# visinf/style-seqcvae

Measured on AMD Instinct MI355X. Metric: captions/sec (train step), higher is better.
Workload: dtype f32; 1 GPU; C2 train step: fwd+bwd+allreduce+clip+SGD, B=64/GPU, R=36, F=2048, L=20 (T=21), Z=128, V=10000, E=1000, H=1200, A=768, SENTIMENT_VAE=1; global_batch=64, parallelism=dp1

## Files before the change

### include/ssc.h

```cpp
#ifndef SSC_H
#define SSC_H

#include <stddef.h>
#include <stdint.h>

#ifdef __cplusplus
extern "C" {
#endif

#define SSC_OK 0
#define SSC_EINVAL (-1)
#define SSC_EALIGN (-2)
#define SSC_EHIP (-3)
#define SSC_EWORKSPACE (-4)

#define SSC_MAX_SEG 6

int ssc_version(void);
int ssc_last_hip_error(void);
const char* ssc_arch(void);

typedef struct {
  const float* A; const float* B;
  int lda, ldb, K;
// ... 14 lines not shown
  const int* m_count; const int* a_rows; const int* c_rows;
  const int* k_count; const int* ka_rows; const int* kb_rows;
  const float* a_scale; const float* b_scale;
  float* topk_part;
} ssc_gemm_desc;

int ssc_pow2_scale(const float* x, size_t rows, int cols, size_t ld, int target_log2, float* out, int combine, float* scratch,
                   void* stream);

int ssc_split_f16(const float* x, int rows, int K, int ldx, const float* scale, void* out, int ldo, const int* row_list,
                  const int* row_count, void* stream);

int ssc_gemm(const ssc_gemm_desc* d, void* stream);

int ssc_gemm_dw_group(const ssc_gemm_desc* const* d, int n, void* stream);

int ssc_set_gemm_mode(int mode);
int ssc_gemm_auto_splits(int M, int N, int ksteps);

int ssc_feat_prep(const float* feats, int B, int R, int F, float* mask, float* avg, void* stream);

int ssc_prep_tokens(const int64_t* caps, int B, int L, int pad, int boundary, int64_t* tokens_tm, float* w_tm,
                    float* nvalid, void* stream);

int ssc_embed_gather(const float* table, int ldt, const int64_t* ids, int n, int E, float* out, int ldo, void* stream);
int ssc_embed_scatter_add(float* dtable, int ldt, const int64_t* ids, int n, int E, const float* d, int ldd, int pad,
                          void* stream);

typedef struct {
  int B, H;
// ... 548 lines not shown
```

### include/ssc_debug.h

```cpp
#ifndef SSC_DEBUG_H
#define SSC_DEBUG_H

#ifdef __cplusplus
extern "C" {
#endif

int ssc_prof_enable(int on);
int ssc_prof_collect(float* out, int max_records);

int ssc_prof_loop_enable(int on);
int ssc_prof_loop_ms(float* fwd_loop_ms, float* bwd_loop_ms);

int ssc_debug_set(const char* key, int value);
int ssc_debug_get(const char* key, int* value);

#ifdef __cplusplus
}
#endif
#endif
```

### style-seqcvae_amd/csrc/gemm.hip

```cpp
#include <stdio.h>
#include <stdlib.h>
#include <string.h>

#include "ssc_common.h"
#include "ssc_debug.h"

typedef float f32x16 __attribute__((ext_vector_type(16)));

namespace {

constexpr int BM = 64, BN = 64, BK = 32;
constexpr int KC_LD = BK + 4;

struct KSeg {
  const float* A;
  const float* B;
  int lda, ldb, K, nsteps;
  int avec, bvec;
  const float* A16;
  const float* B16;
  int lda16, ldb16;
};

struct KArgs {
// ... 1489 lines not shown
    a.seg.s.A16 = a.seg.s.B16 = nullptr; a.seg.s.lda16 = a.seg.s.ldb16 = 0;
    a.nseg = 1; a.M = m.M; a.N = m.N;
    a.out = m.C; a.ldo = m.ldc; a.slab_stride = 0; a.bias = nullptr; a.accumulate = m.accumulate;
    a.steps_total = a.steps_per_split = a.seg.s.nsteps;
    a.mcount = a.arows = a.crows = nullptr;
    a.kcount = m.kcount; a.karows = m.karows; a.kbrows = m.kbrows;
    a.tile_gm = g.tile_gm; a.store_wt = g.store_wt; a.member = p;
    a.topk = nullptr; a.a_scale = a.b_scale = nullptr;
    const int gx = (m.N + 127) / 128, gy = (m.M + 127) / 128;
    const int local = t - m.first;
    x3w_body<false, false, true, 128, 128, PF, NPW>(a, local % gx, local / gx, 0, gx, gy, 1, thr);
    __syncthreads();
  }
}

__global__ void reduce_slabs_kernel(const float* __restrict__ slabs, int nslab, size_t slab_stride, int M, int N,
                                    float* __restrict__ C, int ldc, const float* __restrict__ bias, int accumulate,
                                    const int* __restrict__ mcount, const int* __restrict__ crows) {
  size_t i = (size_t)blockIdx.x * blockDim.x + threadIdx.x;
  if (mcount) M = min(M, *mcount);
  size_t total = (size_t)M * N;
  if (i >= total) return;
  int row = (int)(i / N), col = (int)(i % N);
  float v = 0.f;
  for (int s0 = 0; s0 < nslab; s0 += 8) {
    float t[8];
#pragma unroll
    for (int u = 0; u < 8; ++u) t[u] = slabs[(size_t)min(s0 + u, nslab - 1) * slab_stride + i];
#pragma unroll
    for (int u = 0; u < 8; ++u) v += (s0 + u < nslab) ? t[u] : 0.f;
// ... 198 lines not shown
enum { X3W_NT, X3W_NN, X3W_TN, X3W_TN_KG, X3W_NT_F16_4, X3W_NT_F16_8, X3W_SKINNY_NT, X3W_SKINNY_NN, X3W_FORMS };
const X3wForm g_x3w[X3W_FORMS] = {
    x3w_form<true, true, false, 128, 128, 2, 8>("128x128"), x3w_form<true, false, false, 128, 128, 2, 8>("128x128"),
    x3w_form<false, false, false, 128, 128, 2, 8>("128x128"), x3w_form<false, false, true, 128, 128, 1, 8>("128x128"),
    x3w_form<true, true, false, 128, 128, 2, 4, true>("128x128 f16"), x3w_form<true, true, false, 128, 128, 2, 8, true>("128x128 f16"),
    x3w_form<true, true, false, 64, 256, 2, 8>("64x256"), x3w_form<true, false, false, 64, 256, 2, 8>("64x256"),
};
inline const X3wForm& x3w_big(bool a_kc, bool b_kc, bool kg) {
  return g_x3w[(a_kc && b_kc) ? X3W_NT : a_kc ? X3W_NN : kg ? X3W_TN_KG : X3W_TN];
}
inline const X3wForm& x3w_skinny_form(bool b_kc) { return g_x3w[b_kc ? X3W_SKINNY_NT : X3W_SKINNY_NN]; }

typedef void (*tn_list_fn)(const KTnList);
const tn_list_fn g_tn_list_fn = gemm_x3w_kernel_tn_list<1, 8>;
constexpr int TN_LIST_THREADS = 256 + 64 * 8, TN_LIST_LDS = x3w_lds_bytes<128, 128>();
int g_cus[64] = {};

int x3w_prepare() {
  static bool done_dev[64] = {};
  int dev = 0;
  if (hipGetDevice(&dev) != hipSuccess || dev < 0 || dev >= 64) return SSC_EHIP;
  bool& done = done_dev[dev];
  if (done) return SSC_OK;
  for (const X3wForm& f : g_x3w)
    if (hipFuncSetAttribute((const void*)f.fn, hipFuncAttributeMaxDynamicSharedMemorySize, f.lds) != hipSuccess) return SSC_EHIP;
  if (hipFuncSetAttribute((const void*)g_tn_list_fn, hipFuncAttributeMaxDynamicSharedMemorySize, TN_LIST_LDS) != hipSuccess) return SSC_EHIP;
  if (hipDeviceGetAttribute(&g_cus[dev], hipDeviceAttributeMultiprocessorCount, dev) != hipSuccess || g_cus[dev] < 1) return SSC_EHIP;
  done = true;
  return SSC_OK;
}

inline bool x3w_span_ok(const ssc_gemm_desc* d) {
  const size_t lim = (size_t)1 << 30;
  if (d->ka_rows || d->kb_rows)
    for (int i = 0; i < d->nseg; ++i)
      if (d->seg[i].lda >= (1 << 22) || d->seg[i].ldb >= (1 << 22) || d->seg[i].K >= (1 << 24)) return false;
  for (int i = 0; i < d->nseg; ++i) {
    const size_t K = (size_t)d->seg[i].K;
    if (K == 0) continue;
    const size_t sa = d->a_kc ? (size_t)(d->M - 1) * d->seg[i].lda + K : (K - 1) * d->seg[i].lda + d->M;
    const size_t sb = d->b_kc ? (size_t)(d->N - 1) * d->seg[i].ldb + K : (K - 1) * d->seg[i].ldb + d->N;
// ... 6 lines not shown
}
inline bool vec_all(const KArgs& k) {
  for (int i = 0; i < k.nseg; ++i)
    if (!k.seg[i].avec || !k.seg[i].bvec) return false;
  return true;
}
inline bool x3w_ok(const ssc_gemm_desc* d, const KArgs& k, Num num) {
  return num != Num::F32 && vec_all(k) && (d->a_kc || !d->b_kc) && x3w_span_ok(d);
}

struct Form {
  gemm_fn fn = nullptr;
  const X3wForm* x3w = nullptr;
  dim3 grid;
};
int plan(const ssc_gemm_desc* d, const KArgs& k, int splits, Num num, Form& f) {
  const bool x3 = num != Num::F32, vec = vec_all(k);
  const bool mlist = k.mcount || k.arows || k.crows, klist = k.kcount || k.karows || k.kbrows;
  const bool compact = mlist || klist;
  if (k.topk && !(x3 && vec && d->a_kc && d->b_kc && splits == 1 && !klist && x3w_span_ok(d))) return SSC_EINVAL;
  if (compact) {
    if (!vec) return SSC_EALIGN;
    if (!x3 || (!d->a_kc && d->b_kc)) return SSC_EINVAL;
    if (klist && (k.nseg != 1 || d->a_kc || d->b_kc)) return SSC_EINVAL;
    if (mlist && !d->a_kc) return SSC_EINVAL;
  }
  if (!compact && !k.topk && x3w_skinny_layout(d) && x3w_skinny_shape(d->M, d->N, num) && x3w_ok(d, k, num)) {
    f.x3w = &x3w_skinny_form(d->b_kc);
    f.grid = dim3(ssc_cdiv(d->N, 256), ssc_cdiv(d->M, 64), splits);
    return SSC_OK;
  }
  if (x3 && vec && (d->a_kc || !d->b_kc) && (compact || k.topk || (g_x3b && big_tile(d->M, d->N)))) {
    f.grid = dim3(ssc_cdiv(d->N, 128), ssc_cdiv(d->M, 128), splits);
    const bool kg = k.karows || k.kbrows;
    const long wgs = (long)f.grid.x * f.grid.y * f.grid.z;
    const bool f16 = num == Num::X3_F16 && d->a_kc && d->b_kc && !kg && g_x3b != 3;
    const bool x3w = k.topk || g_x3b == 2 || (g_x3b == 1 && (f16 || wgs >= 768 || (d->M < 512 && big_tile(d->M, d->N))));
    if (x3w && x3w_span_ok(d) && (!kg || (k.karows && k.kbrows))) {
      f.x3w = f16 ? &g_x3w[g_f16_npw == 4 ? X3W_NT_F16_4 : X3W_NT_F16_8] : &x3w_big(d->a_kc, d->b_kc, kg);
      return SSC_OK;
    }
    f.fn = (d->a_kc && d->b_kc) ? gemm_x3b_kernel<true, true, false>
           : d->a_kc            ? gemm_x3b_kernel<true, false, false>
           : kg                 ? gemm_x3b_kernel<false, false, true>
                                : gemm_x3b_kernel<false, false, false>;
    return SSC_OK;
  }
  if (x3 && vec && d->a_kc && d->b_kc) {
    f.fn = gemm_x3_kernel;
    f.grid = dim3(ssc_cdiv(d->N, 64), ssc_cdiv(d->M, 64), splits);
    return SSC_OK;
  }
// ... 332 lines not shown
    *reinterpret_cast<u32x2*>(o + 16) = lo;
  }
}
}
extern "C" int ssc_split_f16(const float* x, int rows, int K, int ldx, const float* scale, void* out, int ldo, const int* row_list,
                             const int* row_count, void* stream) {
  const int kp = ssc_cdiv(K, BK) * BK;
  if (!x || !out || rows <= 0 || K <= 0 || ldx < K || ldo < kp || (ldo & 3) || !ssc_aligned16(out) || (row_list != nullptr) != (row_count != nullptr))
    return SSC_EINVAL;
  SSC_LAUNCH(split_f16_kernel, dim3(ssc_cdiv(kp / 4, 256), rows < 65535 ? rows : 65535), dim3(256), 0, (hipStream_t)stream, x, rows, K, ldx, scale,
             static_cast<unsigned*>(out), ldo, row_list, row_count);
  SSC_CHECK_LAUNCH();
  return SSC_OK;
}

extern "C" int ssc_gemm(const ssc_gemm_desc* d, void* stream) {
  hipStream_t st = (hipStream_t)stream;
  KArgs k;
  SSC_TRY(build_args(d, k));
  if (d->topk_part) {
    k.out = nullptr; k.ldo = d->N; k.slab_stride = 0; k.bias = d->bias; k.accumulate = 0;
    return launch(d, k, 1, st);
  }
  if (!d->C || d->ldc < d->N) return SSC_EINVAL;
  int splits = d->splits;
  if (splits <= 0) splits = ssc_gemm_auto_splits(d->M, d->N, k.steps_total);
  if (splits > k.steps_total) splits = k.steps_total;
  {
    int per = ssc_cdiv(k.steps_total, splits);
    splits = ssc_cdiv(k.steps_total, per);
  }
  if (splits > 1 && (!d->workspace || d->workspace_floats < (size_t)splits * d->M * d->N)) {
    if (d->splits > 1) return SSC_EWORKSPACE;
    splits = d->workspace ? (int)(d->workspace_floats / ((size_t)d->M * d->N)) : 1;
    if (splits < 1) splits = 1;
    int per = ssc_cdiv(k.steps_total, splits);
    splits = ssc_cdiv(k.steps_total, per);
  }
  if (splits == 1) {
    k.out = d->C;
    k.ldo = d->ldc;
    k.slab_stride = 0;
    k.bias = d->bias;
    k.accumulate = d->accumulate;
    return launch(d, k, 1, st);
  }
  k.out = d->workspace;
  k.ldo = d->N;
  k.slab_stride = (size_t)d->M * d->N;
  k.bias = nullptr;
  k.accumulate = 0;
  k.crows = nullptr;
  SSC_TRY(launch(d, k, splits, st));
  size_t total = (size_t)d->M * d->N;
  SSC_LAUNCH(reduce_slabs_kernel, dim3((unsigned)((total + 255) / 256)), dim3(256), 0, st, d->workspace, splits,
                     k.slab_stride, d->M, d->N, d->C, d->ldc, d->bias, d->accumulate, d->m_count, d->c_rows);
  SSC_CHECK_LAUNCH();
  return SSC_OK;
}

extern "C" int ssc_prof_enable(int on) {
  if (on && !g_prof) {
    g_prof = new ProfRec[PROF_MAX];
    for (int i = 0; i < PROF_MAX; ++i) {
      if (hipEventCreate(&g_prof[i].e0) != hipSuccess || hipEventCreate(&g_prof[i].e1) != hipSuccess) return SSC_EHIP;
    }
  }
  if (on && !g_prof_counts && hipHostMalloc((void**)&g_prof_counts, PROF_SLOTS * sizeof(int), hipHostMallocDefault) != hipSuccess) return SSC_EHIP;
  g_prof_on = on != 0;
  if (on) { g_prof_n = 0; g_prof_slots = 0; }
  return SSC_OK;
}
// ... 28 lines not shown
  if (mode == 0 || mode == 1) g_gemm_mode = mode;
  return prev;
}

extern int ssc_g_dec_att_table, ssc_g_dec_dedup, ssc_g_beam_reg, ssc_g_dec_ungathered, ssc_g_dec_parts, ssc_g_dec_planes;
extern int ssc_g_img_mfma;
extern int ssc_g_dw_one_flush;
extern int ssc_g_stream_nt;
namespace {
struct DebugKey { const char* name; int* var; };
const DebugKey g_debug_keys[] = {
    {"large_form", &g_x3b},
    {"x3w_skinny", &g_x3w_skinny},
    {"store_wt", &g_store_wt},
    {"tile_gm", &g_tile_gm},
    {"dw_one_flush", &ssc_g_dw_one_flush},
    {"dec_dedup", &ssc_g_dec_dedup},
    {"beam_reg", &ssc_g_beam_reg},
    {"img_mfma", &ssc_g_img_mfma},
    {"dec_ungathered", &ssc_g_dec_ungathered},
    {"dec_planes", &ssc_g_dec_planes},
    {"dec_parts", &ssc_g_dec_parts},
    {"dec_att_table", &ssc_g_dec_att_table},
    {"f16_npw", &g_f16_npw},
    {"stream_nt", &ssc_g_stream_nt},
    {"gemm_f16", &g_gemm_f16},
};
}

extern "C" int ssc_debug_set(const char* key, int value) {
// ... 20 lines not shown
```

### style-seqcvae_amd/csrc/sequence.hip

```cpp
#include <cstdlib>
#include <initializer_list>

#include "sample_draw.h"
#include "ssc_common.h"
#include "ssc_debug.h"

namespace {

inline size_t r4(size_t x) { return (x + 3) & ~(size_t)3; }

struct Layout {
  int B, R, L, T;
  int V, E, H, A, F, Z, S, tied;
  int Ep, Hp, Ap, Fp, Zp, Vp, H4, XW;
  int D, Dp, SC, NX;
  size_t wc_e, wc_d, pool, dpm;
  size_t total = 0;
  size_t act;
  size_t live;
  size_t tok, w, nvalid, sent_all, wcol_e, wcol_d, mask, avg, pv, emb, ga_static, ga_avg;
  size_t h1, c1, he, ce, hd, cd, gates_a, gates_e, gates_d, q, attn_logits, alpha, att, mu, lv, z, mulv;
  size_t slabs, slab_floats, logits, lse, proj;
  size_t nllw0, nll;
  size_t kld_raw, fb_kdim, fb_gdim, fb_gstep, fb_acc;
// ... 135 lines not shown
  ssc_gemm_desc d;
  fill_desc(d, true, b_kc, segs, M, N);
  d.C = C; d.ldc = ldc; d.bias = bias; d.accumulate = 0;
  d.splits = 0;
  d.workspace = c.slabs; d.workspace_floats = c.slab_floats;
  if (c.act_rows) {
    const int* cnt = live ? c.live_count : c.act_count;
    const int* rows = live ? c.live_rows : c.act_rows;
    d.m_count = cnt; d.a_rows = rows; d.c_rows = rows;
    const int rc = ssc_gemm(&d, c.st);
    if (rc != SSC_EALIGN && rc != SSC_EINVAL) return rc;
    d.m_count = d.a_rows = d.c_rows = nullptr;
  }
  return ssc_gemm(&d, c.st);
}
struct DwBatch {
  static constexpr int MAX = 24;
  ssc_gemm_desc d[MAX];
  int n = 0;
};
int queue_dw(const Ctx& c, DwBatch& q, const float* A, int lda, const float* Bm, int ldb, int K, int M, int N, float* C, int ldc) {
  if (q.n >= DwBatch::MAX) return SSC_EINVAL;
  ssc_gemm_desc& d = q.d[q.n++];
  fill_desc(d, false, false, {{A, lda, Bm, ldb, K}}, M, N);
  d.C = C; d.ldc = ldc;
  d.splits = 0;
  d.workspace = c.slabs; d.workspace_floats = c.slab_floats;
  if (c.live_rows) { d.k_count = c.live_count; d.ka_rows = c.live_rows; d.kb_rows = c.live_rows; }
  return SSC_OK;
}
// ... 252 lines not shown
  Ctx c{st, W + l.slabs, l.slab_floats};
  const int B = l.B, R = l.R, T = l.T, E = l.E, H = l.H, A = l.A, F = l.F, Z = l.Z, S = l.S, V = l.V, H4 = l.H4;
  const int TB = T * B;
  int64_t* tok = (int64_t*)(W + l.tok);
  const size_t sH = (size_t)B * l.Hp;
  const bool fb_on = free_bits > 0.f;

  SSC_TRY(ssc_prep_tokens(bt->caps, B, l.L, cfg->pad, cfg->boundary, tok, W + l.w, W + l.nvalid, st));
  int* act = (int*)(W + l.act);
  int* live = (int*)(W + l.live);
  SSC_LAUNCH(build_active_rows_kernel, dim3(2), dim3(1024), 0, st, W + l.w, TB, B, act, live);
  SSC_CHECK_LAUNCH();
  c.act_count = act; c.act_rows = act + 4;
  c.live_count = live; c.live_rows = live + 4;
  SSC_TRY(ssc_feat_prep(bt->feats, B, R, F, W + l.mask, W + l.avg, st));
  SSC_TRY(gemm(c, true, true, {{bt->feats, F, p->wv, p->ld_wv, F}}, B * R, A, W + l.pv, A));
  const int hoisted = ss_on ? B : TB;
  SSC_TRY(ssc_embed_gather(p->emb, p->ld_emb, tok, hoisted, E, W + l.emb, l.Ep, st));
  SSC_TRY(gemm(c, true, true, {{W + l.emb, l.Ep, p->att_w_ih, p->ld_att_w_ih, E}}, hoisted, H4, W + l.ga_static, H4));
  int64_t* fed_ids = (int64_t*)(W + l.fed_ids);
  if (ss_on && hipMemcpyAsync(fed_ids, tok, (size_t)B * sizeof(int64_t), hipMemcpyDeviceToDevice, st) != hipSuccess) return SSC_EHIP;
  SSC_TRY(gemm(c, true, true, {{W + l.avg, F, p->att_w_ih + E, p->ld_att_w_ih, F}}, B, H4, W + l.ga_avg, H4));
  {
    FillList f;
    for (size_t off : {l.h1, l.c1, l.he, l.ce, l.hd, l.cd}) f.add(W + off, sH);
    f.add(kld, (size_t)B);
    if (fb_on) {
      f.add(W + l.kld_raw, (size_t)B);
      if (free_bits_mode == 3) f.add(W + l.fb_acc, (size_t)B * l.Zp);
    }
    if (l.Zp != Z) {
      f.add(W + l.z, (size_t)TB * l.Zp); f.add(W + l.mu, (size_t)TB * l.Zp); f.add(W + l.lv, (size_t)TB * l.Zp);
    }
    if (cfg->tied) f.add(W + l.proj, (size_t)TB * l.Ep);
// ... 462 lines not shown
  }

  if (g_loop.on) { (void)hipEventRecord(g_loop.e[3], st); g_loop.bwd = true; }

  if (S == 1 && !l.D) {
    SSC_LAUNCH(repeat_kernel, dim3(ssc_cdiv(TB, 256)), dim3(256), 0, st, bt->sentiment, B, T, W + l.sent_all);
    SSC_CHECK_LAUNCH();
  }
  }

  const int zcol = F + 2 * H + S;
  const float* dga = W + l.dga; const float* dge = W + l.dge; const float* dgd = W + l.dgd;
  const float* h1_prev = W + l.h1; const float* h1_new = W + l.h1 + sH;
  const float* hd_prev = W + l.hd; const float* he_prev = W + l.he; const float* he_new = W + l.he + sH;
  const float* att = W + l.att;
  if (phases & 64u) {
  if (g->emb && !cfg->tied) {
    SSC_TRY(ssc_fill(W + l.demb, (size_t)TB * l.Ep, 0.f, st));
    SSC_TRY(gemm_rows(c, false, {{dga, H4, p->att_w_ih, p->ld_att_w_ih, H4}}, TB, E, W + l.demb, l.Ep, nullptr, true));
    if (hipMemset2DAsync(g->emb, (size_t)g->ld_emb * sizeof(float), 0, (size_t)E * sizeof(float), V, st) != hipSuccess)
      return SSC_EHIP;
    SSC_TRY(ssc_embed_scatter_add(g->emb, g->ld_emb, fed_inputs ? (const int64_t*)(W + l.fed_ids) : tok, TB, E, W + l.demb, l.Ep,
                                  cfg->pad, st));
  }
  }
  auto queue_att = [&](DwBatch& q) -> int {
    if (g->att_w_ih) {
      float* gw = g->att_w_ih; int ld = g->ld_att_w_ih;
      SSC_TRY(queue_dw(c, q, dga, H4, W + l.emb, l.Ep, TB, H4, E, gw, ld));
      SSC_TRY(queue_dw(c, q, dga, H4, h1_prev, l.Hp, TB, H4, H, gw + E + F, ld));
      SSC_TRY(queue_dw(c, q, dga, H4, hd_prev, l.Hp, TB, H4, H, gw + E + F + H, ld));
    } else if (g->att_w_hh) {
      SSC_TRY(queue_dw(c, q, dga, H4, h1_prev, l.Hp, TB, H4, H, g->att_w_hh, g->ld_att_w_hh));
    }
    if (g->wq) SSC_TRY(queue_dw(c, q, W + l.dq, l.Ap, h1_new, l.Hp, TB, A, H, g->wq, g->ld_wq));
    return SSC_OK;
  };
  auto queue_enc = [&](DwBatch& q) -> int {
// ... 29 lines not shown
      SSC_TRY(queue_dw(c, q, dgd, H4, hd_prev, l.Hp, TB, H4, H, g->dec_w_hh, g->ld_dec_w_hh));
    }
    return SSC_OK;
  };
  if (one_flush) {
    SSC_TRY(queue_att(dwq));
    SSC_TRY(queue_enc(dwq));
    SSC_TRY(queue_dec(dwq));
    SSC_TRY(flush_dw(c, dwq));
  }
  if (phases & 128u) {
  if (!one_flush) {
    SSC_TRY(queue_att(dwq));
    SSC_TRY(flush_dw(c, dwq));
  }
  if (g->att_w_ih) {
    float* gw = g->att_w_ih; int ld = g->ld_att_w_ih;
    SSC_TRY(gemm(c, false, false, {{W + l.dga_sum, H4, W + l.avg, F, B}}, H4, F, gw + E, ld));
  }
  if (g->att_w_hh) {
    if (g->att_w_ih) {
      if (hipMemcpy2DAsync(g->att_w_hh, (size_t)g->ld_att_w_hh * sizeof(float), g->att_w_ih + E + F,
                           (size_t)g->ld_att_w_ih * sizeof(float), (size_t)H * sizeof(float), H4, hipMemcpyDeviceToDevice,
                           st) != hipSuccess)
        return SSC_EHIP;
    }
  }
  if (g->att_b_ih && g->att_b_hh) {
    SSC_TRY(ssc_colsum2(dga, H4, TB, H4, nullptr, g->att_b_ih, 1, g->att_b_hh, 0, c.slabs, st));
  } else {
    if (g->att_b_ih) SSC_TRY(ssc_colsum2(dga, H4, TB, H4, nullptr, g->att_b_ih, 1, nullptr, 0, c.slabs, st));
    if (g->att_b_hh) SSC_TRY(ssc_colsum2(dga, H4, TB, H4, nullptr, g->att_b_hh, 1, nullptr, 0, c.slabs, st));
  }
  if (g->wv) SSC_TRY(gemm(c, false, false, {{W + l.dpv, A, bt->feats, F, B * R}}, A, F, g->wv, g->ld_wv));
  if (g->wa) SSC_TRY(ssc_colsum(W + l.dwa, A, B, A, nullptr, g->wa, 1, 0, st));
  }
  if (phases & 4u) {
  if (!one_flush) {
    SSC_TRY(queue_enc(dwq));
    SSC_TRY(flush_dw(c, dwq));
  }
  if (g->enc_w_ih) {
    float* gw = g->enc_w_ih; int ld = g->ld_enc_w_ih;
    if (S == 1 && !l.D) SSC_TRY(ssc_colsum2(dge, H4, TB, H4, W + l.sent_all, gw + F + 2 * H, ld, nullptr, 0, c.slabs, st));
    if (l.D && hipMemcpy2DAsync(gw + F + 2 * H, (size_t)ld * sizeof(float), W + l.wc_e, (size_t)l.Dp * sizeof(float),
                                (size_t)l.SC * sizeof(float), H4, hipMemcpyDeviceToDevice, st) != hipSuccess)
      return SSC_EHIP;
  }
  if (g->enc_b_ih && g->enc_b_hh) {
// ... 81 lines not shown
```

### style-seqcvae_amd/ssc_runtime/lib.py

```python
import ctypes as C
import os

_HERE = os.path.dirname(os.path.abspath(__file__))
DEBUG_ENV = os.environ.get("SSC_DEBUG", "") == "1"
LIB_PATH = (DEBUG_ENV and os.environ.get("SSC_LIB_PATH")) or os.path.join(os.path.dirname(_HERE), "libssc_hip.so")
SSC_MAX_SEG = 6

c_float_p = C.POINTER(C.c_float)
c_i64_p = C.POINTER(C.c_int64)
vp = C.c_void_p


class SscError(RuntimeError):
    CODES = {-1: "SSC_EINVAL", -2: "SSC_EALIGN", -3: "SSC_EHIP", -4: "SSC_EWORKSPACE"}

    def __init__(self, fn, rc, hip=0):
        super().__init__(f"{fn} failed: {self.CODES.get(rc, rc)}" + (f" (hipError {hip})" if rc == -3 else ""))
        self.rc = rc


class GemmSeg(C.Structure):
    _fields_ = [("A", vp), ("B", vp), ("lda", C.c_int), ("ldb", C.c_int), ("K", C.c_int),
                ("A16", vp), ("B16", vp), ("lda16", C.c_int), ("ldb16", C.c_int)]

# ... 174 lines not shown

class ScstDesc(C.Structure):
    _fields_ = [("P", C.c_int), ("N", C.c_int), ("steps", C.c_int), ("L", C.c_int), ("end_index", C.c_int), ("predictions", vp),
                ("scores", vp), ("base_scores", vp), ("reward_weights", C.c_double * 6), ("baseline", C.c_int),
                ("loss_scale", C.c_double), ("kld_scale", C.c_double), ("caps", vp), ("lengths", vp), ("reward", vp),
                ("advantage", vp), ("gl", vp), ("gk", vp), ("stats", vp)]


_i, _f, _sz = C.c_int, C.c_float, C.c_size_t
SYMBOLS = {
    "ssc_version": (_i, []),
    "ssc_last_hip_error": (_i, []),
    "ssc_arch": (C.c_char_p, []),
    "ssc_gemm": (_i, [C.POINTER(GemmDesc), vp]),
    "ssc_gemm_dw_group": (_i, [C.POINTER(C.POINTER(GemmDesc)), _i, vp]),
    "ssc_gemm_auto_splits": (_i, [_i, _i, _i]),
    "ssc_pow2_scale": (_i, [vp, _sz, _i, _sz, _i, vp, _i, vp, vp]),
    "ssc_split_f16": (_i, [vp, _i, _i, _i, vp, vp, _i, vp, vp, vp]),
    "ssc_decode_planes_ld": (_i, [vp]),
    "ssc_set_gemm_mode": (_i, [_i]),
    "ssc_feat_prep": (_i, [vp, _i, _i, _i, vp, vp, vp]),
    "ssc_prep_tokens": (_i, [vp, _i, _i, _i, _i, vp, vp, vp, vp]),
    "ssc_embed_gather": (_i, [vp, _i, vp, _i, _i, vp, _i, vp]),
    "ssc_embed_scatter_add": (_i, [vp, _i, vp, _i, _i, vp, _i, _i, vp]),
    "ssc_lstm_fwd": (_i, [C.POINTER(LstmFwdDesc), vp]),
    "ssc_lstm_fwd_z": (_i, [C.POINTER(LstmFwdDesc), vp, _i, vp, _i, _i, vp]),
    "ssc_lstm_fwd_p": (_i, [C.POINTER(LstmFwdDesc), vp, _i, _i, vp, vp]),
    "ssc_lstm_fwd_img": (_i, [C.POINTER(LstmFwdDesc), vp, _i, vp, _i, _i, vp]),
    "ssc_lstm_bwd_x": (_i, [C.POINTER(LstmBwdDesc), vp, _i, vp, _i, _i, vp]),
    "ssc_lstm_bwd": (_i, [C.POINTER(LstmBwdDesc), vp]),
# ... 104 lines not shown
    "ssc_eval_score": (_i, [C.POINTER(EvalRefs), C.POINTER(EvalScoreDesc), vp, _sz, vp]),
    "ssc_eval_set_workspace_bytes": (_sz, [C.POINTER(EvalRefs), C.POINTER(EvalSetDesc)]),
    "ssc_eval_set": (_i, [C.POINTER(EvalRefs), C.POINTER(EvalSetDesc), vp, _sz, vp]),
    "ssc_l2_normalize_rows": (_i, [vp, _i, _i, _i, vp, _i, vp]),
    "ssc_knn_merge": (_i, [vp, _i, _i, _i, _i, _i, vp, vp, vp, vp]),
    "ssc_eval_consensus_workspace_bytes": (_sz, [C.POINTER(EvalRefs), C.POINTER(EvalConsensusDesc)]),
    "ssc_eval_consensus": (_i, [C.POINTER(EvalRefs), C.POINTER(EvalConsensusDesc), vp, _sz, vp]),
    "ssc_scst_prepare": (_i, [C.POINTER(ScstDesc), vp]),
}

DEBUG_SYMBOLS = {
    "ssc_prof_enable": (_i, [_i]),
    "ssc_prof_collect": (_i, [vp, _i]),
    "ssc_prof_loop_enable": (_i, [_i]),
    "ssc_prof_loop_ms": (_i, [C.POINTER(C.c_float), C.POINTER(C.c_float)]),
    "ssc_debug_set": (_i, [C.c_char_p, _i]),
    "ssc_debug_get": (_i, [C.c_char_p, C.POINTER(C.c_int)]),
}

_lib = None


class _Lib:
    def __init__(self, cdll):
        self._cdll = cdll
        for name, (res, args) in list(SYMBOLS.items()) + list(DEBUG_SYMBOLS.items()):
            fn = getattr(cdll, name)
            fn.restype = res
            fn.argtypes = args
            setattr(self, "_raw_" + name, fn)
# ... 39 lines not shown
```

Before: 7996 captions/s.

## Batch independent large GEMMs into one persistent grouped list kernel

Adds a grouped GEMM list kernel that runs several independent large x3w 128x128 GEMMs in one persistent launch, with tiles ordered by steps per split. It is used for the forward visual-projection and embedding-input GEMMs and for three backward weight-gradient GEMMs (embedding grad, att_w_ih avg part, wv). The aim is to cut launch count and fill the CUs better when single GEMMs underfill the device. In exchange it forces the x3w form for listed GEMMs, carves split-K workspace per member, and moves the embedding scatter later in the backward pass.

```diff
diff --git a/include/ssc.h b/include/ssc.h
--- a/include/ssc.h
+++ b/include/ssc.h
@@ -52,6 +52,8 @@
 int ssc_gemm(const ssc_gemm_desc* d, void* stream);
 
 int ssc_gemm_dw_group(const ssc_gemm_desc* const* d, int n, void* stream);
+
+int ssc_gemm_list(const ssc_gemm_desc* const* d, int n, void* stream);
 
 int ssc_set_gemm_mode(int mode);
 int ssc_gemm_auto_splits(int M, int N, int ksteps);
diff --git a/include/ssc_debug.h b/include/ssc_debug.h
--- a/include/ssc_debug.h
+++ b/include/ssc_debug.h
@@ -1,5 +1,7 @@
 #ifndef SSC_DEBUG_H
 #define SSC_DEBUG_H
+
+#include "ssc.h"
 
 #ifdef __cplusplus
 extern "C" {
@@ -11,6 +13,8 @@
 int ssc_prof_loop_enable(int on);
 int ssc_prof_loop_ms(float* fwd_loop_ms, float* bwd_loop_ms);
 
+int ssc_debug_list_plan(const ssc_gemm_desc* const* d, int n, int* out);
+
 int ssc_debug_set(const char* key, int value);
 int ssc_debug_get(const char* key, int* value);
 
diff --git a/style-seqcvae_amd/csrc/gemm.hip b/style-seqcvae_amd/csrc/gemm.hip
--- a/style-seqcvae_amd/csrc/gemm.hip
+++ b/style-seqcvae_amd/csrc/gemm.hip
@@ -1527,6 +1527,37 @@
   }
 }
 
+enum { LIST_NT = 0, LIST_NN = 1, LIST_TN = 2, LIST_TN_KG = 3 };
+struct KList {
+  KArgs a[SSC_GROUP_MAX];
+  int n, total;
+  int first[SSC_GROUP_MAX + 1];
+  int gx[SSC_GROUP_MAX], gy[SSC_GROUP_MAX], gz[SSC_GROUP_MAX], lay[SSC_GROUP_MAX];
+};
+template <int NPW>
+__global__ __launch_bounds__(256 + 64 * NPW, 1) void gemm_x3w_kernel_list(const KList g) {
+  int p = 0;
+  for (int t = blockIdx.x; t < g.total; t += gridDim.x) {
+#pragma unroll 1
+    while (p + 1 < g.n && t >= g.first[p + 1]) ++p;
+    int thr = (int)threadIdx.x;
+    asm volatile("" : "+v"(thr));
+    __builtin_assume(thr >= 0 && thr < 256 + 64 * NPW);
+    const KArgs& a = g.a[p];
+    const int gx = g.gx[p], gy = g.gy[p], gz = g.gz[p];
+    const int local = t - g.first[p];
+    const int x = local % gx, yz = local / gx;
+    const int y = yz % gy, z = yz / gy;
+    switch (g.lay[p]) {
+      case LIST_NT: x3w_body<true, true, false, 128, 128, 2, NPW>(a, x, y, z, gx, gy, gz, thr); break;
+      case LIST_NN: x3w_body<true, false, false, 128, 128, 2, NPW>(a, x, y, z, gx, gy, gz, thr); break;
+      case LIST_TN: x3w_body<false, false, false, 128, 128, 2, NPW>(a, x, y, z, gx, gy, gz, thr); break;
+      default: x3w_body<false, false, true, 128, 128, 1, NPW>(a, x, y, z, gx, gy, gz, thr); break;
+    }
+    __syncthreads();
+  }
+}
+
 __global__ void reduce_slabs_kernel(const float* __restrict__ slabs, int nslab, size_t slab_stride, int M, int N,
                                     float* __restrict__ C, int ldc, const float* __restrict__ bias, int accumulate,
                                     const int* __restrict__ mcount, const int* __restrict__ crows) {
@@ -1755,6 +1786,8 @@
 typedef void (*tn_list_fn)(const KTnList);
 const tn_list_fn g_tn_list_fn = gemm_x3w_kernel_tn_list<1, 8>;
 constexpr int TN_LIST_THREADS = 256 + 64 * 8, TN_LIST_LDS = x3w_lds_bytes<128, 128>();
+typedef void (*list_fn)(const KList);
+const list_fn g_list_fn = gemm_x3w_kernel_list<8>;
 int g_cus[64] = {};
 
 int x3w_prepare() {
@@ -1766,6 +1799,7 @@
   for (const X3wForm& f : g_x3w)
     if (hipFuncSetAttribute((const void*)f.fn, hipFuncAttributeMaxDynamicSharedMemorySize, f.lds) != hipSuccess) return SSC_EHIP;
   if (hipFuncSetAttribute((const void*)g_tn_list_fn, hipFuncAttributeMaxDynamicSharedMemorySize, TN_LIST_LDS) != hipSuccess) return SSC_EHIP;
+  if (hipFuncSetAttribute((const void*)g_list_fn, hipFuncAttributeMaxDynamicSharedMemorySize, TN_LIST_LDS) != hipSuccess) return SSC_EHIP;
   if (hipDeviceGetAttribute(&g_cus[dev], hipDeviceAttributeMultiprocessorCount, dev) != hipSuccess || g_cus[dev] < 1) return SSC_EHIP;
   done = true;
   return SSC_OK;
@@ -1802,7 +1836,8 @@
   const X3wForm* x3w = nullptr;
   dim3 grid;
 };
-int plan(const ssc_gemm_desc* d, const KArgs& k, int splits, Num num, Form& f) {
+int plan(const ssc_gemm_desc* d, const KArgs& k, int splits, Num num, Form& f, int large_form = -1) {
+  const int x3b = large_form >= 0 ? large_form : g_x3b;
   const bool x3 = num != Num::F32, vec = vec_all(k);
   const bool mlist = k.mcount || k.arows || k.crows, klist = k.kcount || k.karows || k.kbrows;
   const bool compact = mlist || klist;
@@ -1818,12 +1853,12 @@
     f.grid = dim3(ssc_cdiv(d->N, 256), ssc_cdiv(d->M, 64), splits);
     return SSC_OK;
   }
-  if (x3 && vec && (d->a_kc || !d->b_kc) && (compact || k.topk || (g_x3b && big_tile(d->M, d->N)))) {
+  if (x3 && vec && (d->a_kc || !d->b_kc) && (compact || k.topk || (x3b && big_tile(d->M, d->N)))) {
     f.grid = dim3(ssc_cdiv(d->N, 128), ssc_cdiv(d->M, 128), splits);
     const bool kg = k.karows || k.kbrows;
     const long wgs = (long)f.grid.x * f.grid.y * f.grid.z;
-    const bool f16 = num == Num::X3_F16 && d->a_kc && d->b_kc && !kg && g_x3b != 3;
-    const bool x3w = k.topk || g_x3b == 2 || (g_x3b == 1 && (f16 || wgs >= 768 || (d->M < 512 && big_tile(d->M, d->N))));
+    const bool f16 = num == Num::X3_F16 && d->a_kc && d->b_kc && !kg && x3b != 3;
+    const bool x3w = k.topk || x3b == 2 || (x3b == 1 && (f16 || wgs >= 768 || (d->M < 512 && big_tile(d->M, d->N))));
     if (x3w && x3w_span_ok(d) && (!kg || (k.karows && k.kbrows))) {
       f.x3w = f16 ? &g_x3w[g_f16_npw == 4 ? X3W_NT_F16_4 : X3W_NT_F16_8] : &x3w_big(d->a_kc, d->b_kc, kg);
       return SSC_OK;
@@ -2186,6 +2221,110 @@
   return SSC_OK;
 }
 
+int ssc_g_large_list = ssc_env_int("SSC_LARGE_LIST", 1);
+namespace {
+int resolve_output(const ssc_gemm_desc* d, KArgs& k, int& splits) {
+  if (!d->C || d->ldc < d->N) return SSC_EINVAL;
+  splits = d->splits;
+  if (splits <= 0) splits = ssc_gemm_auto_splits(d->M, d->N, k.steps_total);
+  if (splits > k.steps_total) splits = k.steps_total;
+  {
+    int per = ssc_cdiv(k.steps_total, splits);
+    splits = ssc_cdiv(k.steps_total, per);
+  }
+  if (splits > 1 && (!d->workspace || d->workspace_floats < (size_t)splits * d->M * d->N)) {
+    if (d->splits > 1) return SSC_EWORKSPACE;
+    splits = d->workspace ? (int)(d->workspace_floats / ((size_t)d->M * d->N)) : 1;
+    if (splits < 1) splits = 1;
+    int per = ssc_cdiv(k.steps_total, splits);
+    splits = ssc_cdiv(k.steps_total, per);
+  }
+  if (splits == 1) {
+    k.out = d->C;
+    k.ldo = d->ldc;
+    k.slab_stride = 0;
+    k.bias = d->bias;
+    k.accumulate = d->accumulate;
+    return SSC_OK;
+  }
+  k.out = d->workspace;
+  k.ldo = d->N;
+  k.slab_stride = (size_t)d->M * d->N;
+  k.bias = nullptr;
+  k.accumulate = 0;
+  k.crows = nullptr;
+  return SSC_OK;
+}
+int reduce_output(const ssc_gemm_desc* d, const KArgs& k, int splits, hipStream_t st) {
+  size_t total = (size_t)d->M * d->N;
+  SSC_LAUNCH(reduce_slabs_kernel, dim3((unsigned)((total + 255) / 256)), dim3(256), 0, st, d->workspace, splits,
+                     k.slab_stride, d->M, d->N, d->C, d->ldc, d->bias, d->accumulate, d->m_count, d->c_rows);
+  SSC_CHECK_LAUNCH();
+  return SSC_OK;
+}
+
+inline bool ranges_overlap(const float* a, size_t na, const float* b, size_t nb) { return a < b + nb && b < a + na; }
+int list_layout(const ssc_gemm_desc* d, const KArgs& k, int splits, Num num) {
+  if (num != Num::X3 || g_x3b == 0 || g_x3b == 3 || k.topk || d->M < BIG_MIN_M) return -1;
+  Form f;
+  if (plan(d, k, splits, num, f, 2) != SSC_OK || !f.x3w) return -1;
+  for (int lay = LIST_NT; lay <= LIST_TN_KG; ++lay)
+    if (f.x3w == &g_x3w[lay]) return lay;
+  return -1;
+}
+static_assert(X3W_NT == LIST_NT && X3W_NN == LIST_NN && X3W_TN == LIST_TN && X3W_TN_KG == LIST_TN_KG, "list bodies follow g_x3w");
+struct ListPlan {
+  KArgs k[SSC_GROUP_MAX];
+  int splits[SSC_GROUP_MAX], lay[SSC_GROUP_MAX];
+};
+void build_list(const ListPlan& lp, int n, KList& g, int* ord) {
+  for (int i = 0; i < n; ++i) ord[i] = i;
+  for (int i = 1; i < n; ++i)
+    for (int j = i; j > 0 && lp.k[ord[j]].steps_per_split > lp.k[ord[j - 1]].steps_per_split; --j) { const int t = ord[j]; ord[j] = ord[j - 1]; ord[j - 1] = t; }
+  g.n = n;
+  g.first[0] = 0;
+  for (int i = 0; i < n; ++i) {
+    const int s = ord[i];
+    g.a[i] = lp.k[s];
+    g.a[i].member = i;
+    g.lay[i] = lp.lay[s];
+    g.gx[i] = ssc_cdiv(lp.k[s].N, 128); g.gy[i] = ssc_cdiv(lp.k[s].M, 128); g.gz[i] = lp.splits[s];
+    g.first[i + 1] = g.first[i] + g.gx[i] * g.gy[i] * g.gz[i];
+  }
+  for (int i = n; i < SSC_GROUP_MAX; ++i) { g.first[i + 1] = g.first[n]; g.gx[i] = g.gy[i] = g.gz[i] = 1; g.lay[i] = LIST_NT; }
+  g.total = g.first[n];
+}
+int launch_list(const ListPlan& lp, const ssc_gemm_desc* const* d, int n, hipStream_t st) {
+  SSC_TRY(x3w_prepare());
+  int dev = 0;
+  if (hipGetDevice(&dev) != hipSuccess) return SSC_EHIP;
+  KList g;
+  memset(&g, 0, sizeof(g));
+  int ord[SSC_GROUP_MAX];
+  build_list(lp, n, g, ord);
+  const ssc_gemm_desc* ds[SSC_GROUP_MAX];
+  int Kmax = 0, Nmax = 0;
+  long MN = 0;
+  bool one_layout = true;
+  for (int i = 0; i < n; ++i) {
+    ds[i] = d[ord[i]];
+    int K = 0;
+    for (int s = 0; s < ds[i]->nseg; ++s) K += ds[i]->seg[s].K;
+    if (K > Kmax) Kmax = K;
+    if (ds[i]->N > Nmax) Nmax = ds[i]->N;
+    MN += (long)ds[i]->M * ds[i]->N;
+    one_layout = one_layout && g.lay[i] == g.lay[0];
+  }
+  ProfRec* rec = prof_open(ds, n, (int)(MN / Nmax), Nmax, Kmax, g.gz[0], st);
+  if (one_layout) SSC_AUDIT_BEGIN();
+  SSC_LAUNCH(g_list_fn, dim3(g.total < g_cus[dev] ? g.total : g_cus[dev]), dim3(TN_LIST_THREADS), TN_LIST_LDS, st, g);
+  if (one_layout) SSC_AUDIT_END(g.a, n, g.lay[0] <= LIST_NN, g.lay[0] == LIST_NT, "128x128 list", st);
+  prof_close(rec, st);
+  SSC_CHECK_LAUNCH();
+  return SSC_OK;
+}
+}
+
 extern "C" int ssc_gemm(const ssc_gemm_desc* d, void* stream) {
   hipStream_t st = (hipStream_t)stream;
   KArgs k;
@@ -2194,40 +2333,84 @@
     k.out = nullptr; k.ldo = d->N; k.slab_stride = 0; k.bias = d->bias; k.accumulate = 0;
     return launch(d, k, 1, st);
   }
-  if (!d->C || d->ldc < d->N) return SSC_EINVAL;
-  int splits = d->splits;
-  if (splits <= 0) splits = ssc_gemm_auto_splits(d->M, d->N, k.steps_total);
-  if (splits > k.steps_total) splits = k.steps_total;
-  {
-    int per = ssc_cdiv(k.steps_total, splits);
-    splits = ssc_cdiv(k.steps_total, per);
-  }
-  if (splits > 1 && (!d->workspace || d->workspace_floats < (size_t)splits * d->M * d->N)) {
-    if (d->splits > 1) return SSC_EWORKSPACE;
-    splits = d->workspace ? (int)(d->workspace_floats / ((size_t)d->M * d->N)) : 1;
-    if (splits < 1) splits = 1;
-    int per = ssc_cdiv(k.steps_total, splits);
-    splits = ssc_cdiv(k.steps_total, per);
-  }
-  if (splits == 1) {
-    k.out = d->C;
-    k.ldo = d->ldc;
-    k.slab_stride = 0;
-    k.bias = d->bias;
-    k.accumulate = d->accumulate;
-    return launch(d, k, 1, st);
-  }
-  k.out = d->workspace;
-  k.ldo = d->N;
-  k.slab_stride = (size_t)d->M * d->N;
-  k.bias = nullptr;
-  k.accumulate = 0;
-  k.crows = nullptr;
+  int splits = 1;
+  SSC_TRY(resolve_output(d, k, splits));
+  if (splits == 1) return launch(d, k, 1, st);
   SSC_TRY(launch(d, k, splits, st));
-  size_t total = (size_t)d->M * d->N;
-  SSC_LAUNCH(reduce_slabs_kernel, dim3((unsigned)((total + 255) / 256)), dim3(256), 0, st, d->workspace, splits,
-                     k.slab_stride, d->M, d->N, d->C, d->ldc, d->bias, d->accumulate, d->m_count, d->c_rows);
-  SSC_CHECK_LAUNCH();
+  return reduce_output(d, k, splits, st);
+}
+
+namespace {
+constexpr int LIST_NMAX = 32, LIST_CALL_MAX = (LIST_NMAX + SSC_GROUP_MAX - 1) / SSC_GROUP_MAX;
+struct ListCall {
+  int nlists = 0;
+  ListPlan lp[LIST_CALL_MAX];
+  int ln[LIST_CALL_MAX];
+  int src[LIST_CALL_MAX][SSC_GROUP_MAX];
+  int list_of[LIST_NMAX];
+};
+void plan_lists(const ssc_gemm_desc* const* d, int n, Num num, ListCall& c) {
+  int cur = 0;
+  c.ln[0] = 0;
+  for (int j = 0; j < n; ++j) {
+    c.list_of[j] = -1;
+    if (!ssc_g_large_list) continue;
+    KArgs k;
+    int splits = 1;
+    if (build_args(d[j], k) != SSC_OK || d[j]->topk_part || resolve_output(d[j], k, splits) != SSC_OK) continue;
+    k.steps_per_split = ssc_cdiv(k.steps_total, splits);
+    const int lay = list_layout(d[j], k, splits, num);
+    if (lay < 0) continue;
+    ListPlan& lp = c.lp[cur];
+    int& ln = c.ln[cur];
+    bool shared = false;
+    for (int i = 0; i < ln && splits > 1; ++i)
+      shared = shared || (lp.splits[i] > 1 && ranges_overlap(k.out, (size_t)splits * k.slab_stride, lp.k[i].out, (size_t)lp.splits[i] * lp.k[i].slab_stride));
+    if (shared) continue;
+    lp.k[ln] = k; lp.splits[ln] = splits; lp.lay[ln] = lay; c.src[cur][ln] = j;
+    c.list_of[j] = cur;
+    if (++ln == SSC_GROUP_MAX) c.ln[++cur] = 0;
+  }
+  c.nlists = cur + (c.ln[cur] ? 1 : 0);
+}
+}
+
+extern "C" int ssc_gemm_list(const ssc_gemm_desc* const* d, int n, void* stream) {
+  hipStream_t st = (hipStream_t)stream;
+  if (!d || n < 1 || n > LIST_NMAX) return SSC_EINVAL;
+  for (int j = 0; j < n; ++j)
+    if (!d[j]) return SSC_EINVAL;
+  ListCall c;
+  plan_lists(d, n, numerics(), c);
+  for (int q = 0; q < c.nlists; ++q) {
+    const ssc_gemm_desc* ld[SSC_GROUP_MAX];
+    for (int i = 0; i < c.ln[q]; ++i) ld[i] = d[c.src[q][i]];
+    SSC_TRY(launch_list(c.lp[q], ld, c.ln[q], st));
+    for (int i = 0; i < c.ln[q]; ++i)
+      if (c.lp[q].splits[i] > 1) SSC_TRY(reduce_output(ld[i], c.lp[q].k[i], c.lp[q].splits[i], st));
+  }
+  for (int j = 0; j < n; ++j)
+    if (c.list_of[j] < 0) SSC_TRY(ssc_gemm(d[j], stream));
+  return SSC_OK;
+}
+
+extern "C" int ssc_debug_list_plan(const ssc_gemm_desc* const* d, int n, int* out) {
+  if (!d || !out || n < 1 || n > LIST_NMAX) return SSC_EINVAL;
+  for (int j = 0; j < n; ++j)
+    if (!d[j]) return SSC_EINVAL;
+  ListCall c;
+  plan_lists(d, n, numerics(), c);
+  for (int j = 0; j < n; ++j) { int* o = out + 6 * j; o[0] = -1; o[1] = o[2] = o[3] = o[4] = o[5] = 0; }
+  for (int q = 0; q < c.nlists; ++q) {
+    KList g;
+    memset(&g, 0, sizeof(g));
+    int ord[SSC_GROUP_MAX];
+    build_list(c.lp[q], c.ln[q], g, ord);
+    for (int i = 0; i < c.ln[q]; ++i) {
+      int* o = out + 6 * c.src[q][ord[i]];
+      o[0] = q; o[1] = i; o[2] = g.first[i]; o[3] = g.first[i + 1] - g.first[i]; o[4] = g.lay[i]; o[5] = g.a[i].steps_per_split;
+    }
+  }
   return SSC_OK;
 }
 
@@ -2286,6 +2469,7 @@
     {"x3w_skinny", &g_x3w_skinny},
     {"store_wt", &g_store_wt},
     {"tile_gm", &g_tile_gm},
+    {"large_list", &ssc_g_large_list},
     {"dw_one_flush", &ssc_g_dw_one_flush},
     {"dec_dedup", &ssc_g_dec_dedup},
     {"beam_reg", &ssc_g_beam_reg},
diff --git a/style-seqcvae_amd/csrc/sequence.hip b/style-seqcvae_amd/csrc/sequence.hip
--- a/style-seqcvae_amd/csrc/sequence.hip
+++ b/style-seqcvae_amd/csrc/sequence.hip
@@ -4,6 +4,8 @@
 #include "sample_draw.h"
 #include "ssc_common.h"
 #include "ssc_debug.h"
+
+extern int ssc_g_large_list;
 
 namespace {
 
@@ -173,6 +175,45 @@
   }
   return ssc_gemm(&d, c.st);
 }
+struct BigBatch {
+  static constexpr int MAX = 4;
+  ssc_gemm_desc d[MAX];
+  int n = 0;
+  size_t used = 0;
+};
+int queue_big(const Ctx& c, BigBatch& q, bool a_kc, bool b_kc, Seg s, int M, int N, float* C, int ldc, bool live_rows) {
+  if (q.n >= BigBatch::MAX) return SSC_EINVAL;
+  ssc_gemm_desc& d = q.d[q.n++];
+  fill_desc(d, a_kc, b_kc, {s}, M, N);
+  d.C = C; d.ldc = ldc;
+  d.splits = 0;
+  const int splits = ssc_gemm_auto_splits(M, N, ssc_cdiv(s.K, 32));
+  const size_t want = splits > 1 ? (size_t)splits * M * N : 0;
+  if (q.used + want <= c.slab_floats) { d.workspace = c.slabs + q.used; d.workspace_floats = want; q.used += (want + 3) & ~(size_t)3; }
+  else { d.workspace = c.slabs; d.workspace_floats = c.slab_floats; }
+  if (live_rows && c.live_rows) { d.m_count = c.live_count; d.a_rows = c.live_rows; d.c_rows = c.live_rows; }
+  return SSC_OK;
+}
+int flush_big(const Ctx& c, BigBatch& q) {
+  if (!q.n) return SSC_OK;
+  const ssc_gemm_desc* dp[BigBatch::MAX];
+  for (int i = 0; i < q.n; ++i) dp[i] = &q.d[i];
+  auto issue = [&]() -> int {
+    if (ssc_g_large_list == 2) {
+      for (int i = 0; i < q.n; ++i) SSC_TRY(ssc_gemm(dp[i], c.st));
+      return SSC_OK;
+    }
+    return ssc_gemm_list(dp, q.n, c.st);
+  };
+  int rc = issue();
+  if (rc == SSC_EALIGN || rc == SSC_EINVAL) {
+    bool had = false;
+    for (int i = 0; i < q.n; ++i) { had = had || q.d[i].m_count; q.d[i].m_count = q.d[i].a_rows = q.d[i].c_rows = nullptr; }
+    if (had) rc = issue();
+  }
+  q.n = 0; q.used = 0;
+  return rc;
+}
 struct DwBatch {
   static constexpr int MAX = 24;
   ssc_gemm_desc d[MAX];
@@ -455,10 +496,19 @@
   c.act_count = act; c.act_rows = act + 4;
   c.live_count = live; c.live_rows = live + 4;
   SSC_TRY(ssc_feat_prep(bt->feats, B, R, F, W + l.mask, W + l.avg, st));
-  SSC_TRY(gemm(c, true, true, {{bt->feats, F, p->wv, p->ld_wv, F}}, B * R, A, W + l.pv, A));
   const int hoisted = ss_on ? B : TB;
   SSC_TRY(ssc_embed_gather(p->emb, p->ld_emb, tok, hoisted, E, W + l.emb, l.Ep, st));
-  SSC_TRY(gemm(c, true, true, {{W + l.emb, l.Ep, p->att_w_ih, p->ld_att_w_ih, E}}, hoisted, H4, W + l.ga_static, H4));
+  {
+    ssc_gemm_desc dl[2];
+    fill_desc(dl[0], true, true, {{bt->feats, F, p->wv, p->ld_wv, F}}, B * R, A);
+    dl[0].C = W + l.pv; dl[0].ldc = A;
+    fill_desc(dl[1], true, true, {{W + l.emb, l.Ep, p->att_w_ih, p->ld_att_w_ih, E}}, hoisted, H4);
+    dl[1].C = W + l.ga_static; dl[1].ldc = H4;
+    for (ssc_gemm_desc& d : dl) { d.splits = 0; d.workspace = c.slabs; d.workspace_floats = c.slab_floats; }
+    const ssc_gemm_desc* dp[2] = {&dl[0], &dl[1]};
+    if (ssc_g_large_list == 3) { SSC_TRY(ssc_gemm(dp[0], st)); SSC_TRY(ssc_gemm(dp[1], st)); }
+    else SSC_TRY(ssc_gemm_list(dp, 2, st));
+  }
   int64_t* fed_ids = (int64_t*)(W + l.fed_ids);
   if (ss_on && hipMemcpyAsync(fed_ids, tok, (size_t)B * sizeof(int64_t), hipMemcpyDeviceToDevice, st) != hipSuccess) return SSC_EHIP;
   SSC_TRY(gemm(c, true, true, {{W + l.avg, F, p->att_w_ih + E, p->ld_att_w_ih, F}}, B, H4, W + l.ga_avg, H4));
@@ -951,14 +1001,23 @@
   const float* h1_prev = W + l.h1; const float* h1_new = W + l.h1 + sH;
   const float* hd_prev = W + l.hd; const float* he_prev = W + l.he; const float* he_new = W + l.he + sH;
   const float* att = W + l.att;
-  if (phases & 64u) {
-  if (g->emb && !cfg->tied) {
-    SSC_TRY(ssc_fill(W + l.demb, (size_t)TB * l.Ep, 0.f, st));
-    SSC_TRY(gemm_rows(c, false, {{dga, H4, p->att_w_ih, p->ld_att_w_ih, H4}}, TB, E, W + l.demb, l.Ep, nullptr, true));
+  BigBatch bigq;
+  const bool emb_grad = (phases & 64u) && g->emb && !cfg->tied;
+  const bool emb_joins = emb_grad && (phases & 128u);
+  auto scatter_emb = [&]() -> int {
     if (hipMemset2DAsync(g->emb, (size_t)g->ld_emb * sizeof(float), 0, (size_t)E * sizeof(float), V, st) != hipSuccess)
       return SSC_EHIP;
-    SSC_TRY(ssc_embed_scatter_add(g->emb, g->ld_emb, fed_inputs ? (const int64_t*)(W + l.fed_ids) : tok, TB, E, W + l.demb, l.Ep,
-                                  cfg->pad, st));
+    return ssc_embed_scatter_add(g->emb, g->ld_emb, fed_inputs ? (const int64_t*)(W + l.fed_ids) : tok, TB, E, W + l.demb, l.Ep,
+                                 cfg->pad, st);
+  };
+  if (phases & 64u) {
+  if (emb_grad) {
+    SSC_TRY(ssc_fill(W + l.demb, (size_t)TB * l.Ep, 0.f, st));
+    SSC_TRY(queue_big(c, bigq, true, false, {dga, H4, p->att_w_ih, p->ld_att_w_ih, H4}, TB, E, W + l.demb, l.Ep, true));
+    if (!emb_joins) {
+      SSC_TRY(flush_big(c, bigq));
+      SSC_TRY(scatter_emb());
+    }
   }
   }
   auto queue_att = [&](DwBatch& q) -> int {
@@ -1018,10 +1077,10 @@
     SSC_TRY(queue_att(dwq));
     SSC_TRY(flush_dw(c, dwq));
   }
-  if (g->att_w_ih) {
-    float* gw = g->att_w_ih; int ld = g->ld_att_w_ih;
-    SSC_TRY(gemm(c, false, false, {{W + l.dga_sum, H4, W + l.avg, F, B}}, H4, F, gw + E, ld));
-  }
+  if (g->att_w_ih) SSC_TRY(queue_big(c, bigq, false, false, {W + l.dga_sum, H4, W + l.avg, F, B}, H4, F, g->att_w_ih + E, g->ld_att_w_ih, false));
+  if (g->wv) SSC_TRY(queue_big(c, bigq, false, false, {W + l.dpv, A, bt->feats, F, B * R}, A, F, g->wv, g->ld_wv, false));
+  SSC_TRY(flush_big(c, bigq));
+  if (emb_joins) SSC_TRY(scatter_emb());
   if (g->att_w_hh) {
     if (g->att_w_ih) {
       if (hipMemcpy2DAsync(g->att_w_hh, (size_t)g->ld_att_w_hh * sizeof(float), g->att_w_ih + E + F,
@@ -1036,7 +1095,6 @@
     if (g->att_b_ih) SSC_TRY(ssc_colsum2(dga, H4, TB, H4, nullptr, g->att_b_ih, 1, nullptr, 0, c.slabs, st));
     if (g->att_b_hh) SSC_TRY(ssc_colsum2(dga, H4, TB, H4, nullptr, g->att_b_hh, 1, nullptr, 0, c.slabs, st));
   }
-  if (g->wv) SSC_TRY(gemm(c, false, false, {{W + l.dpv, A, bt->feats, F, B * R}}, A, F, g->wv, g->ld_wv));
   if (g->wa) SSC_TRY(ssc_colsum(W + l.dwa, A, B, A, nullptr, g->wa, 1, 0, st));
   }
   if (phases & 4u) {
diff --git a/style-seqcvae_amd/ssc_runtime/lib.py b/style-seqcvae_amd/ssc_runtime/lib.py
--- a/style-seqcvae_amd/ssc_runtime/lib.py
+++ b/style-seqcvae_amd/ssc_runtime/lib.py
@@ -212,6 +212,7 @@
     "ssc_arch": (C.c_char_p, []),
     "ssc_gemm": (_i, [C.POINTER(GemmDesc), vp]),
     "ssc_gemm_dw_group": (_i, [C.POINTER(C.POINTER(GemmDesc)), _i, vp]),
+    "ssc_gemm_list": (_i, [C.POINTER(C.POINTER(GemmDesc)), _i, vp]),
     "ssc_gemm_auto_splits": (_i, [_i, _i, _i]),
     "ssc_pow2_scale": (_i, [vp, _sz, _i, _sz, _i, vp, _i, vp, vp]),
     "ssc_split_f16": (_i, [vp, _i, _i, _i, vp, vp, _i, vp, vp, vp]),
@@ -346,6 +347,7 @@
     "ssc_prof_collect": (_i, [vp, _i]),
     "ssc_prof_loop_enable": (_i, [_i]),
     "ssc_prof_loop_ms": (_i, [C.POINTER(C.c_float), C.POINTER(C.c_float)]),
+    "ssc_debug_list_plan": (_i, [C.POINTER(C.POINTER(GemmDesc)), _i, C.POINTER(C.c_int)]),
     "ssc_debug_set": (_i, [C.c_char_p, _i]),
     "ssc_debug_get": (_i, [C.c_char_p, C.POINTER(C.c_int)]),
 }
```

Measured after the change: 8036 captions/s (median of 6 runs). Within noise of the previous version (+0.5%).
